# sringe/CatINT

Measured on AMD Instinct MI355X. Metric: batched 1D PNP Newton-timesteps/sec, higher is better.
Workload: dtype f64; 1 GPU; BASELINE configs[1]: batch=1024 operating points/GPU, 3 species, 512 grid points, fp64, Crank-Nicolson compat integrator, Dirichlet-Dirichlet Poisson; batch_per_gpu=1024, nspecies=3, nx=512, steps_per_launch=256, parallelism=batch-sharded x1

## Files before the change

### catint_amd/csrc/pnp_kernels.hip

```cpp
#include "pnp_internal.h"
#include "pnp_wave.h"

namespace pnp {

template <int P, bool WANT_V, int SHIFT, bool DD = false>
__device__ __forceinline__ double poisson_wave(const DevArgs& A, double* LV, double* GV, double* VV, double* X,
                                               double vw, double vb, double gw, double gb, int lane) {
  const int nx = A.nx, m = A.m;
  const int r0 = lane * P;
  const double dx = A.dx;
  double vown[P], gown[P];
  double v1;
  if constexpr (!WANT_V && P >= 2) {
    if (DD || A.pb_mode == PNP_PB_DD) {
      double Hi[P];
      const double dx2 = A.dx2;
      double s0 = 0.0, s1 = 0.0;
      double hm1, hm2, h0, h1, incT, incW;
      if constexpr (DD) {
        if (lane == 0) LV[pidx<P>(nx - 1)] = 0.0;
        lds_sync();
        {
#pragma clang fp contract(off)
#pragma unroll
          for (int j = 0; j < P; ++j) Hi[j] = LV[pidx<P>(r0 + j + 1)] * dx2;
          hm1 = LV[pidx<P>(m)] * dx2;
          hm2 = LV[pidx<P>(m - 1)] * dx2;
          h0 = LV[pidx<P>(1)] * dx2;
          h1 = LV[pidx<P>(2)] * dx2;
        }
#pragma unroll
        for (int j = 0; j < P; ++j) {
          s0 += Hi[j];
          s1 = __builtin_fma((double)j, Hi[j], s1);
        }
      } else {
#pragma unroll
        for (int j = 0; j < P; ++j) {
          double h = LV[pidx<P>(r0 + j + 1)] * dx2;
          h = (r0 + j == m) ? 0.0 : h;
          Hi[j] = h;
          s0 += h;
          s1 = __builtin_fma((double)j, h, s1);
        }
        hm1 = pick_blocked<P>(Hi, r0, m - 1);
        hm2 = pick_blocked<P>(Hi, r0, m - 2);
        h0 = read_lane(Hi[0], 0);
        h1 = read_lane(Hi[1], 0);
      }
      const double wsum = __builtin_fma((double)(m - r0), s0, -s1);
#pragma unroll
      for (int j = 1; j < P; ++j) Hi[j] += Hi[j - 1];
      if constexpr (DD) {
        incT = wave_scan_incl_bc(Hi[P - 1]);
        incW = wave_scan_incl_bc(wsum);
      } else {
        incT = wave_scan_incl(Hi[P - 1]);
        incW = wave_scan_incl(wsum);
      }
      const double base = from_prev_lane(0.0, incT);
      const double tot1 = read_lane(incT, 63), totG = read_lane(incW, 63);
#pragma unroll
      for (int j = 0; j < P; ++j) Hi[j] += base;
      const double w0 = (vb - vw - totG) / A.nxm1;
      const double inv2dx = A.inv2dx;
#pragma unroll
      for (int j = 0; j < P; ++j) {
        const double Hx = (j == 0) ? base : Hi[j > 0 ? j - 1 : 0];
        GV[pidx<P>(r0 + j + 1 + SHIFT)] = inv2dx * ((w0 + Hi[j]) + (w0 + Hx));
      }
      const double g1 = inv2dx * ((w0 + h0) + (w0 + 0.0));
      const double g2 = inv2dx * ((w0 + (h0 + h1)) + (w0 + h0));
      const double g_first = g1 + (g1 - g2);
      const double Hm1 = tot1 - hm1, Hm2 = Hm1 - hm2;
      const double gm1 = inv2dx * ((w0 + tot1) + (w0 + Hm1));
      const double gm2 = inv2dx * ((w0 + Hm1) + (w0 + Hm2));
      const double g_last = gm1 + (gm1 - gm2);
      lds_sync();
      if (lane == 0) {
        GV[pidx<P>(0 + SHIFT)] = g_first;
        GV[pidx<P>(nx - 1 + SHIFT)] = g_last;
        if constexpr (SHIFT == 1) {
          GV[pidx<P>(0)] = g_first;
          GV[pidx<P>(nx + 1)] = g_last;
          if constexpr (DD) GV[pidx<P>(nx - 2 + 1)] = g_last;
        }
      }
      lds_sync();
      return vw + w0;
    }
  }
  if (A.pb_mode == PNP_PB_DD) {
    double Hi[P];
    const double dx2 = dx * dx;
    if (lane == 0) LV[pidx<P>(nx - 1)] = 0.0;
    lds_sync();
#pragma unroll
    for (int j = 0; j < P; ++j) Hi[j] = LV[pidx<P>(r0 + j + 1)] * dx2;
    double tot1, baseH, totG;
    const double inv2dx = 1.0 / (2 * dx);
    if constexpr (!WANT_V) {
      double wsum = 0.0;
      const double wj0 = (double)(m - r0);
#pragma unroll
      for (int j = 0; j < P; ++j) wsum = __builtin_fma(wj0 - (double)j, Hi[j], wsum);
      blocked_scan_sum<P>(Hi, wsum, X, lane, tot1, baseH, totG);
    } else {
      double G[P];
      blocked_scan<P, false>(Hi, X, lane, tot1, baseH);
#pragma unroll
      for (int j = 0; j < P; ++j) G[j] = Hi[j];
      double totAll, baseG;
      blocked_scan<P, false>(G, X, lane, totAll, baseG);
      totG = totAll - (double)(64 * P - m) * tot1;
      const double w0v = (vb - vw - totG) / (double)(nx - 1);
#pragma unroll
      for (int j = 0; j < P; ++j) {
        const double Gex = (j == 0) ? baseG : G[j > 0 ? j - 1 : 0];
        vown[j] = vw + (double)(r0 + j + 1) * w0v + Gex;
      }
    }
    const double w0 = (vb - vw - totG) / (double)(nx - 1);
#pragma unroll
    for (int j = 0; j < P; ++j) {
      const double Hx = (j == 0) ? baseH : Hi[j > 0 ? j - 1 : 0];
      gown[j] = inv2dx * ((w0 + Hi[j]) + (w0 + Hx));
    }
    v1 = vw + 1.0 * w0 + 0.0;
  } else {
    const bool g_from_wall = (A.pb_mode == PNP_PB_GWALL_VBULK) || (A.pb_mode == PNP_PB_VWALL_GWALL);
    const bool v_from_wall = (A.pb_mode == PNP_PB_VWALL_GBULK) || (A.pb_mode == PNP_PB_VWALL_GWALL);
    double t[P];
#pragma unroll
    for (int j = 0; j < P; ++j) {
      const double lv = LV[pidx<P>(r0 + j + 1)];
      t[j] = (r0 + j < m) ? lv * dx : 0.0;
    }
    double tot, base;
    if (g_from_wall) {
      blocked_scan<P, false>(t, X, lane, tot, base);
#pragma unroll
      for (int j = 0; j < P; ++j) gown[j] = gw + t[j];
    } else {
      blocked_scan<P, true>(t, X, lane, tot, base);
#pragma unroll
      for (int j = 0; j < P; ++j) gown[j] = gb - t[j];
    }
#pragma unroll
    for (int j = 0; j < P; ++j) t[j] = (r0 + j < m) ? gown[j] * dx : 0.0;
    if (v_from_wall) {
      blocked_scan<P, false>(t, X, lane, tot, base);
#pragma unroll
      for (int j = 0; j < P; ++j) vown[j] = vw + t[j];
    } else {
      blocked_scan<P, true>(t, X, lane, tot, base);
#pragma unroll
      for (int j = 0; j < P; ++j) vown[j] = vb - t[j];
    }
    v1 = __shfl(vown[0], 0, 64);
  }
#pragma unroll
  for (int j = 0; j < P; ++j) {
    GV[pidx<P>(r0 + j + 1 + SHIFT)] = gown[j];
    if constexpr (WANT_V) VV[pidx<P>(r0 + j + 1)] = vown[j];
  }
  lds_sync();
  if (lane == 0) {
    const double g1 = GV[pidx<P>(1 + SHIFT)], g2 = GV[pidx<P>(2 + SHIFT)];
    const double gm1 = GV[pidx<P>(nx - 2 + SHIFT)], gm2 = GV[pidx<P>(nx - 3 + SHIFT)];
    double g0, gl;
    if (A.pb_mode == PNP_PB_DD) {
      g0 = g1 + (g1 - g2);
      gl = gm1 + (gm1 - gm2);
    } else if (A.pb_mode == PNP_PB_GWALL_VBULK || A.pb_mode == PNP_PB_VWALL_GWALL) {
      g0 = gw;
      gl = gm1 + (gm1 - gm2);
    } else {
      gl = gb;
      g0 = g1 + (g1 - g2);
    }
    GV[pidx<P>(0 + SHIFT)] = g0;
    GV[pidx<P>(nx - 1 + SHIFT)] = gl;
    if constexpr (SHIFT == 1) {
      GV[pidx<P>(0)] = g0;
      GV[pidx<P>(nx + 1)] = gl;
    }
    if constexpr (WANT_V) {
      const double v1 = VV[pidx<P>(1)], v2 = VV[pidx<P>(2)];
      const double vm1 = VV[pidx<P>(nx - 2)], vm2 = VV[pidx<P>(nx - 3)];
      double v0, vl;
      if (A.pb_mode == PNP_PB_DD) {
        v0 = vw;
        vl = vb;
      } else if (A.pb_mode == PNP_PB_VWALL_GBULK || A.pb_mode == PNP_PB_VWALL_GWALL) {
        v0 = vw;
        vl = vm1 + (vm1 - vm2);
      } else {
        vl = vb;
        v0 = v1 + (v1 - v2);
      }
      VV[pidx<P>(0)] = v0;
      VV[pidx<P>(nx - 1)] = vl;
    }
  }
  lds_sync();
  return v1;
}

template <int P, int G>
constexpr int step_min_waves() {
  return P <= 2 ? 4 : (P == 4 ? (G == 1 ? 4 : 2) : (P == 8 ? (G == 1 ? 3 : 1) : 1));
}

__device__ __forceinline__ double uniform_f64(double v) {
  const int lo = __builtin_amdgcn_readfirstlane(__double2loint(v));
  const int hi = __builtin_amdgcn_readfirstlane(__double2hiint(v));
  return __hiloint2double(hi, lo);
}

template <int P, int W, int G, bool FAST>
__device__ __forceinline__ void step_body(const DevArgs& A, double* lds) {
  constexpr int RB = rowbuf_doubles<P>();
  constexpr int NR = W * G;
  constexpr int V1SLOT = RB - 2;
  constexpr int IT2 = P / (2 * W) + 1;
  const int tid = threadIdx.x;
  const int lane = tid & 63;
  const int wave = __builtin_amdgcn_readfirstlane(tid >> 6);
  const int64_t b = blockIdx.x;
  const int nx = A.nx, m = A.m, ldx = A.ldx, N = A.N;
  double* LV = lds;
  double* GV = lds + RB;
  double* ROWS = lds + 2 * RB;
  double* ROW0 = ROWS + wave * (G * RB);
  const int r0 = lane * P;
  const double dx = A.dx, dt = A.dt;

  double* lin = A.lapl_a + b * (int64_t)ldx;
  double* lout = A.lapl_b + b * (int64_t)ldx;
  double* crow0 = A.c + b * (int64_t)N * ldx;
  const bool single_round = FAST || (N <= NR);
  const bool cn = FAST || (A.method == PNP_METHOD_CRANK_NICOLSON);
  const bool use_mig = FAST || A.use_mig;
  double chk = 0.0;
  double mn = 0.0;
  for (int i = tid; i < (2 + NR) * RB; i += 64 * W) lds[i] = 0.0;
  wg_sync<W>();
  const int ls2 = pidx<P>(2 * tid);
  const bool lead_all = W > 1 && wave == 0 && A.B <= 2048;
  if (lead_all) __builtin_amdgcn_s_setprio(3);

  auto stage_first_round = [&]() {
    RowRegs<P> rl, rr[G];
    if (wave == 0 && use_mig) load_row_issue<P>(row_rsrc(lin, ldx), rl, lane);
    if (wave * G < N) {
#pragma unroll
      for (int g = 0; g < G; ++g)
        load_row_issue<P>(row_rsrc(crow0 + (int64_t)min(wave * G + g, N - 1) * ldx, ldx), rr[g], lane);
    }
    if (wave == 0 && use_mig) load_row_commit<P>(rl, LV, lane);
    if (wave * G < N) {
#pragma unroll
      for (int g = 0; g < G; ++g) load_row_commit<P>(rr[g], ROW0 + g * RB, lane);
    }
    lds_sync();
  };

  double k_vw = 0.0, k_vb = 0.0, k_vz = 0.0;
  double k_f2dx[G], k_cL[G], k_mu[G], k_twoD[G], k_hsr[G], k_e4r[G], k_eer[G], k_omsr[G], k_qe[NR];
  if constexpr (FAST) {
    k_vw = uniform_f64(A.pb[b * 4 + 0]);
    k_vb = uniform_f64(A.pb[b * 4 + 1]);
    k_vz = uniform_f64(A.vzeta[b]);
#pragma unroll
    for (int g = 0; g < G; ++g) {
      const int k = min(wave * G + g, N - 1);
      const SpecConst& S = A.spec[k];
      k_f2dx[g] = uniform_f64(2 * A.flux[b * N + k] * dx);
      k_cL[g] = uniform_f64(A.cbulk[b * N + k]);
      k_mu[g] = uniform_f64(S.mu);
      k_twoD[g] = uniform_f64(S.twoD);
      k_hsr[g] = uniform_f64(S.hsr);
      k_e4r[g] = uniform_f64(S.e4r);
      k_eer[g] = uniform_f64(S.eer);
      k_omsr[g] = uniform_f64(S.omsr);
    }
#pragma unroll
    for (int w2 = 0; w2 < NR; ++w2) k_qe[w2] = uniform_f64(A.spec[min(w2, N - 1)].qe);
    stage_first_round();
  }

  for (int step = 0; step < A.nsteps; ++step) {
    const bool resident = single_round && step > 0;
    const bool last_step = step + 1 == A.nsteps;
    if constexpr (!FAST) {
      if (!resident) stage_first_round();
    }
    __builtin_amdgcn_sched_barrier(0);
    if (use_mig) {
      if (wave == 0) {
        const double vw = FAST ? k_vw : A.pb[b * 4 + 0], vb = FAST ? k_vb : A.pb[b * 4 + 1];
        const double gw = FAST ? 0.0 : A.pb[b * 4 + 2], gb = FAST ? 0.0 : A.pb[b * 4 + 3];
        int lane_o = lane;
        asm volatile("" : "+v"(lane_o));
        if (W > 1 && !lead_all) __builtin_amdgcn_s_setprio(3);
        const double v1w = poisson_wave<P, false, 1, FAST>(A, LV, GV, nullptr, GV, vw, vb, gw, gb, lane_o);
        if (W > 1 && !lead_all) __builtin_amdgcn_s_setprio(0);
        if (lane == 0) {
          GV[V1SLOT] = v1w;
          if (!FAST && cn) GV[pidx<P>(nx - 2 + 1)] = GV[pidx<P>(nx - 1 + 1)];
        }
      }
    }
    wg_sync<W>();
    const double v1 = use_mig ? GV[V1SLOT] : 0.0;
    const double vz = FAST ? k_vz : A.vzeta[b];

    d2 accp[IT2];
#pragma unroll
    for (int it = 0; it < IT2; ++it) accp[it] = (d2)(0.0);

    for (int k0 = 0; k0 < N; k0 = FAST ? N : k0 + NR) {
      const int kw = k0 + wave * G;
      if (kw < N) {
        int kg[G];
#pragma unroll
        for (int g = 0; g < G; ++g) kg[g] = min(kw + g, N - 1);
        if (!FAST && k0 > 0) {
          RowRegs<P> rr[G];
#pragma unroll
          for (int g = 0; g < G; ++g) load_row_issue<P>(row_rsrc(crow0 + (int64_t)kg[g] * ldx, ldx), rr[g], lane);
#pragma unroll
          for (int g = 0; g < G; ++g) load_row_commit<P>(rr[g], ROW0 + g * RB, lane);
          lds_sync();
        }
        double c0new[G], cLv[G], pat0[G], patL[G];
#pragma unroll
        for (int g = 0; g < G; ++g) {
          const double* ROW = ROW0 + g * RB;
          const SpecConst& S = A.spec[kg[g]];
          const double flux = FAST ? 0.0 : A.flux[b * N + kg[g]];
          const double cL = FAST ? k_cL[g] : A.cbulk[b * N + kg[g]];
          const double c1 = ROW[pidx<P>(1)];
          const double c0old = ROW[pidx<P>(0)];
          const double cLold = ROW[pidx<P>(nx - 1)];
          double aa;
          if constexpr (FAST) {
#pragma clang fp contract(off)
            aa = k_mu[g] * (v1 - vz);
          } else {
            aa = S.mu * (v1 - vz);
          }
          if (cn) {
            const double twoD = FAST ? k_twoD[g] : S.twoD;
            const double rden = fast_rcp2(-twoD + aa);
            c0new[g] = (-twoD - aa) * rden * c1 - (FAST ? k_f2dx[g] : 2 * flux * dx) * rden;
          } else {
            c0new[g] = ((S.twoD + aa) * c1 + flux * 2. * dx) * fast_rcp2(S.twoD - aa);
          }
          cLv[g] = cL;
          pat0[g] = cn ? (c0new[g] + c0old) : c0new[g];
          patL[g] = cn ? (cL + cLold) : cL;
        }
        lds_sync();
        if (lane == 0) {
#pragma unroll
          for (int g = 0; g < G; ++g) {
            ROW0[g * RB + pidx<P>(0)] = pat0[g];
            ROW0[g * RB + pidx<P>(nx - 1)] = patL[g];
          }
        }
        lds_sync();
        double x[G][P];
        if (cn) {
          double ta[G][P], tc[G][P];
          {
            const int jmu = (m - 1) % P;
            const bool in_lm = lane == (m - 1) / P;
#pragma unroll
            for (int g = 0; g < G; ++g) {
              const double* ROW = ROW0 + g * RB;
              const SpecConst& S = A.spec[kg[g]];
              const double hsr = FAST ? k_hsr[g] : S.hsr, e4r = FAST ? k_e4r[g] : S.e4r;
              const double eer = FAST ? k_eer[g] : S.eer, omsr = FAST ? k_omsr[g] : S.omsr;
              double cc[P + 2], g4[P + 2];
#pragma unroll
              for (int t = 0; t < P + 2; ++t) cc[t] = ROW[pidx<P>(r0 + t)];
#pragma unroll
              for (int t = 0; t < P + 2; ++t) g4[t] = e4r * GV[pidx<P>(r0 + t)];
#pragma unroll
              for (int j = 0; j < P; ++j) {
                const double lq = LV[pidx<P>(r0 + j)];
                const double left = cc[j] * (hsr + g4[j]);
                const double right = cc[j + 2] * (hsr - g4[j + 2]);
                x[g][j] = left + cc[j + 1] * (omsr + eer * lq) + right;
                ta[g][j] = -hsr + g4[j + 1];
                tc[g][j] = -hsr - g4[j + 1];
                if (j == jmu) tc[g][j] = in_lm ? 0.0 : tc[g][j];
              }
              if (lane == 0) ta[g][0] = 0.0;
            }
          }
          __builtin_amdgcn_sched_barrier(0);
          lds_sync();
          tridiag_wave<P, G, FAST>(ta, tc, x, ROW0, RB, lane);
        } else {
          double gq[P + 2];
#pragma unroll
          for (int t = 0; t < P + 2; ++t) gq[t] = A.use_mig ? GV[pidx<P>(r0 + t + 1)] : 0.0;
#pragma unroll
          for (int g = 0; g < G; ++g) {
            const double* ROW = ROW0 + g * RB;
            const SpecConst& S = A.spec[kg[g]];
            const double sf = S.sf, dm = S.dm, Mf = S.Mf;
            double cc[P + 2];
#pragma unroll
            for (int t = 0; t < P + 2; ++t) cc[t] = ROW[pidx<P>(r0 + t)];
#pragma unroll
            for (int j = 0; j < P; ++j) {
              double Wt = sf - dm * gq[j + 2] + 0.5;
              double Et = sf + dm * gq[j] + 0.5;
              if (!A.lf) {
                Wt -= 0.5;
                Et -= 0.5;
              }
              double val = __builtin_fma(Wt, cc[j + 2], __builtin_fma(Mf, cc[j + 1], Et * cc[j]));
              if (A.has_rates) val += A.rates[(b * N + kg[g]) * (int64_t)ldx + min(r0 + j + 1, nx - 1)] * dt;
              x[g][j] = val;
            }
          }
          lds_sync();
        }
#pragma unroll
        for (int g = 0; g < G; ++g) {
          double* ROW = ROW0 + g * RB;
#pragma unroll
          for (int j = 0; j < P; ++j) ROW[pidx<P>(r0 + j + 1)] = x[g][j];
        }
        lds_sync();
#pragma unroll
        for (int g = 0; g < G; ++g) {
          double* ROW = ROW0 + g * RB;
          if (lane == 0) {
            ROW[pidx<P>(0)] = c0new[g];
            ROW[pidx<P>(nx - 1)] = cLv[g];
          }
          if (lane < ldx - nx) ROW[pidx<P>(nx + lane)] = 0.0;
        }
      }
      wg_sync<W>();
      const int nk = min(NR, N - k0);
      auto store_and_fold = [&](int w2, double qe) {
        const double* R2 = ROWS + w2 * RB;
        double* grow = crow0 + (int64_t)(k0 + w2) * ldx;
        const __amdgpu_buffer_rsrc_t rs = row_rsrc(grow, ldx);
#pragma unroll
        for (int it = 0; it < IT2; ++it) {
          if (FAST && W > 1 && it > 0 && 128 * (W * it + wave) >= ldx) continue;
          const int sl = min(pair_slot<P>(ls2, W * it), RB - 4);
          d2 t;
          t.x = R2[sl];
          t.y = R2[sl + PAIR_STEP<P>];
          __builtin_amdgcn_raw_buffer_store_b128(__builtin_bit_cast(u4, t), rs, tid * 16 + it * (1024 * W), 0, 0);
          accp[it].x = __builtin_fma(-t.x, qe, accp[it].x);
          accp[it].y = __builtin_fma(-t.y, qe, accp[it].y);
          if (last_step) {
            const bool inrow = 2 * tid + 128 * W * it < ldx;
            const double sx = inrow ? t.x : 0.0, sy = inrow ? t.y : 0.0;
            chk += (sx - sx) + (sy - sy);
            mn = fmin(mn, fmin(sx, sy));
          }
        }
      };
      if constexpr (FAST) {
#pragma unroll
        for (int w2 = 0; w2 < NR; ++w2)
          if (w2 < nk) store_and_fold(w2, k_qe[w2]);
      } else {
        for (int w2 = 0; w2 < nk; ++w2) store_and_fold(w2, A.spec[k0 + w2].qe);
        wg_sync<W>();
      }
    }
    const bool keep = single_round && (step + 1 < A.nsteps);
    {
      const __amdgpu_buffer_rsrc_t rs = row_rsrc(lout, ldx);
#pragma unroll
      for (int it = 0; it < IT2; ++it) {
        if (FAST && W > 1 && it > 0 && 128 * (W * it + wave) >= ldx) continue;
        __builtin_amdgcn_raw_buffer_store_b128(__builtin_bit_cast(u4, accp[it]), rs, tid * 16 + it * (1024 * W), 0, 0);
        if (keep && 2 * tid + 128 * W * it < ldx) {
          LV[pair_slot<P>(ls2, W * it)] = accp[it].x;
          LV[pair_slot<P>(ls2, W * it) + PAIR_STEP<P>] = accp[it].y;
        }
      }
    }
    double* tmp = lin;
    lin = lout;
    lout = tmp;
    if (step + 1 < A.nsteps) {
      if (single_round) {
        wg_sync<W>();
      } else {
        __builtin_amdgcn_fence(__ATOMIC_RELEASE, "workgroup");
        if constexpr (W > 1) __builtin_amdgcn_s_barrier();
        __builtin_amdgcn_fence(__ATOMIC_ACQUIRE, "workgroup");
      }
    }
  }
  const unsigned long long nan_mask = __ballot(chk != chk);
  const unsigned long long neg_mask = __ballot(mn < 0.0);
  if (lane == 0) {
    int st = PNP_STATUS_OK;
    if (neg_mask) st = PNP_STATUS_NEGATIVE;
    if (nan_mask) st = PNP_STATUS_NAN;
    if (st) atomicMax(&A.status[b], st);
#ifdef PNP_HWID_PROBE
    const unsigned simd = __builtin_amdgcn_s_getreg((1 << 11) | (4 << 6) | 4);
    unsigned v = 1u << (8 + 4 * wave + simd);
    if (wave == 0) v |= (__builtin_amdgcn_s_getreg((3 << 11) | (8 << 6) | 4) << 20) | (__builtin_amdgcn_s_getreg((2 << 11) | (13 << 6) | 4) << 24);
    atomicOr((unsigned*)&A.status[b], v);
#endif
  }
}

template <int P, int W, int G>
constexpr bool step_has_fast_body() {
  return P >= 2 && !(W == 1 && G == 3 && (P == 2 || P == 16));
}

template <int P, int W, int G>
__global__ __launch_bounds__(64 * W, (step_min_waves<P, G>())) void step_kernel(const DevArgs A) {
  extern __shared__ __attribute__((aligned(16))) double lds[];
  if constexpr (step_has_fast_body<P, W, G>()) {
    const bool fast = A.method == PNP_METHOD_CRANK_NICOLSON && A.use_mig && A.pb_mode == PNP_PB_DD && !A.has_rates &&
                      A.N <= W * G && !A.step_generic;
    if (fast) {
      step_body<P, W, G, true>(A, lds);
      return;
    }
  }
  step_body<P, W, G, false>(A, lds);
}

template <int P, int W>
constexpr int step_rr_min_waves() {
  return P <= 4 ? 4 : (P == 8 ? 3 : 1);
}

template <int P, int W, bool CN>
__global__ __launch_bounds__(64 * W, (step_rr_min_waves<P, W>())) void step_kernel_rr(const DevArgs A) {
  static_assert(P >= 2 && P % 2 == 0, "window loads need an even P");
  extern __shared__ __attribute__((aligned(16))) double lds[];
  constexpr int XS = 384;
  constexpr int PS = 64 * P + 2;
  const int tid = threadIdx.x;
  const int lane = tid & 63;
  const int wave = __builtin_amdgcn_readfirstlane(tid >> 6);
  const int64_t b = blockIdx.x;
  const int nx = A.nx, m = A.m, ldx = A.ldx, N = A.N;
  const int r0 = lane * P;
  const double dx = A.dx;
  constexpr bool cn = CN;
  double* strip = lds + wave * XS;
  double* part = lds + W * XS;
  double* lin = A.lapl_a + b * (int64_t)ldx;
  double* lout = A.lapl_b + b * (int64_t)ldx;
  double* crow0 = A.c + b * (int64_t)N * ldx;
  const double vw = A.pb[b * 4 + 0], vb = A.pb[b * 4 + 1];
  const double vz = A.vzeta[b];
  const bool single_round = (N <= W);
  double chk = 0.0, mn = 0.0;

  double lw[P + 2];
  double cc[P + 2];
  for (int step = 0; step < A.nsteps; ++step) {
    const bool last_step = step + 1 == A.nsteps;
    const bool resident = single_round && step > 0;
    if (!resident) {
      if (A.use_mig) load_window<P>(row_rsrc(lin, ldx), lw, lane);
      load_window<P>(row_rsrc(crow0 + (int64_t)min(wave, N - 1) * ldx, ldx), cc, lane);
    }
    double gx[P + 3];
    double v1 = 0.0;
    if (A.use_mig) {
      double Hi[P];
      const double dx2 = dx * dx;
      double s0 = 0.0, s1 = 0.0;
#pragma unroll
      for (int j = 0; j < P; ++j) {
        double h = lw[j + 1] * dx2;
        h = (r0 + j == m) ? 0.0 : h;
        Hi[j] = h;
        s0 += h;
        s1 = __builtin_fma((double)j, h, s1);
      }
      const double wsum = __builtin_fma((double)(m - r0), s0, -s1);
      const double hm1 = pick_blocked<P>(Hi, r0, m - 1), hm2 = pick_blocked<P>(Hi, r0, m - 2);
      const double h0 = read_lane(Hi[0], 0), h1 = read_lane(Hi[1], 0);
#pragma unroll
      for (int j = 1; j < P; ++j) Hi[j] += Hi[j - 1];
      const double incT = wave_scan_incl(Hi[P - 1]);
      const double incW = wave_scan_incl(wsum);
      const double base = from_prev_lane(0.0, incT);
      const double tot1 = read_lane(incT, 63), totG = read_lane(incW, 63);
#pragma unroll
      for (int j = 0; j < P; ++j) Hi[j] += base;
      const double w0 = (vb - vw - totG) / (double)(nx - 1);
      v1 = vw + w0;
      const double inv2dx = 1.0 / (2 * dx);
      double gown[P];
#pragma unroll
      for (int j = 0; j < P; ++j) {
        const double Hx = (j == 0) ? base : Hi[j > 0 ? j - 1 : 0];
        gown[j] = inv2dx * ((w0 + Hi[j]) + (w0 + Hx));
      }
      const double g1 = inv2dx * ((w0 + h0) + (w0 + 0.0));
      const double g2 = inv2dx * ((w0 + (h0 + h1)) + (w0 + h0));
      const double g_first = g1 + (g1 - g2);
      const double Hm1 = tot1 - hm1, Hm2 = Hm1 - hm2;
      const double gm1 = inv2dx * ((w0 + tot1) + (w0 + Hm1));
      const double gm2 = inv2dx * ((w0 + Hm1) + (w0 + Hm2));
      const double g_last = gm1 + (gm1 - gm2);
#pragma unroll
      for (int t = 2; t < P + 2; ++t) gx[t] = gown[t - 2];
      gx[1] = from_prev_lane(g_first, gown[P - 1]);
      gx[0] = from_prev_lane(g_first, gown[P - 2]);
      gx[P + 2] = from_next_lane(0.0, gown[0]);
#pragma unroll
      for (int t = 2; t < P + 3; ++t) {
        const int idx = r0 - 1 + t;
        gx[t] = ((cn && idx == nx - 2) || idx == nx - 1) ? g_last : gx[t];
      }
    } else {
#pragma unroll
      for (int t = 0; t < P + 3; ++t) gx[t] = 0.0;
    }

    double acc[P];
#pragma unroll
    for (int j = 0; j < P; ++j) acc[j] = 0.0;
    double acc0 = 0.0, accL = 0.0;

    for (int k = wave; k < N; k += W) {
      if (k != wave) load_window<P>(row_rsrc(crow0 + (int64_t)k * ldx, ldx), cc, lane);
      const SpecConst& S = A.spec[k];
      const double flux = A.flux[b * N + k];
      const double cL = A.cbulk[b * N + k];
      const double c0old = read_lane(cc[0], 0);
      const double c1 = read_lane(cc[1], 0);
      const double aa = S.mu * (v1 - vz);
      double c0new;
      if (cn) {
        const double rden = fast_rcp2(-S.twoD + aa);
        c0new = (-S.twoD - aa) * rden * c1 - 2 * flux * dx * rden;
      } else {
        c0new = ((S.twoD + aa) * c1 + flux * 2. * dx) * fast_rcp2(S.twoD - aa);
      }
      const double qe = S.qe;
      const double pat0 = cn ? (c0new + c0old) : c0new;
      const double patL = cn ? (cL + cL) : cL;
      cc[0] = (lane == 0) ? pat0 : cc[0];
#pragma unroll
      for (int t = 2; t < P + 2; ++t) cc[t] = (r0 + t == nx - 1) ? patL : cc[t];
      double x[1][P];
      if (cn) {
        double ta[1][P], tc[1][P];
        const double hsr = S.hsr, e4r = S.e4r, eer = S.eer, omsr = S.omsr;
#pragma unroll
        for (int j = 0; j < P; ++j) {
          const double gm = e4r * gx[j], g0 = e4r * gx[j + 1], gp = e4r * gx[j + 2];
          const double left = cc[j] * (hsr + gm);
          const double right = cc[j + 2] * (hsr - gp);
          x[0][j] = left + cc[j + 1] * (omsr + eer * lw[j]) + right;
          ta[0][j] = -hsr + g0;
          tc[0][j] = (r0 + j == m - 1) ? 0.0 : (-hsr - g0);
        }
        ta[0][0] = (lane == 0) ? 0.0 : ta[0][0];
        tridiag_wave<P, 1>(ta, tc, x, strip, XS, lane);
      } else {
        const double sf = S.sf, dm = S.dm, Mf = S.Mf;
#pragma unroll
        for (int j = 0; j < P; ++j) {
          double Wt = sf - dm * gx[j + 3] + 0.5;
          double Et = sf + dm * gx[j + 1] + 0.5;
          if (!A.lf) {
            Wt -= 0.5;
            Et -= 0.5;
          }
          x[0][j] = Et * cc[j] + Mf * cc[j + 1] + Wt * cc[j + 2];
        }
      }
      double* grow = crow0 + (int64_t)k * ldx;
      store_rows<P>(__builtin_amdgcn_make_buffer_rsrc(grow, 0, (nx - 1) * 8, 0x00020000), x[0], lane);
      if (lane == 0) grow[0] = c0new;
#pragma unroll
      for (int j = 0; j < P; ++j) {
        const double xv = (r0 + j < m) ? x[0][j] : 0.0;
        acc[j] = __builtin_fma(-xv, qe, acc[j]);
        if (last_step) {
          chk += xv - xv;
          mn = fmin(mn, xv);
        }
      }
      if (last_step) {
        chk += c0new - c0new;
        mn = fmin(mn, c0new);
      }
      acc0 = __builtin_fma(-c0new, qe, acc0);
      accL = __builtin_fma(-cL, qe, accL);
      if (single_round) {
#pragma unroll
        for (int j = 0; j < P; ++j) cc[j + 1] = x[0][j];
        cc[0] = from_prev_lane(c0new, x[0][P - 1]);
        cc[P + 1] = from_next_lane(0.0, x[0][0]);
      }
    }
    if constexpr (W > 1) {
      double* mine = part + ((step & 1) * W + wave) * PS;
#pragma unroll
      for (int j = 0; j < P; ++j) mine[r0 + j] = acc[j];
      if (lane == 0) {
        mine[64 * P] = acc0;
        mine[64 * P + 1] = accL;
      }
      wg_sync<W>();
      const double* all = part + (step & 1) * W * PS;
#pragma unroll
      for (int j = 0; j < P; ++j) {
        double t = all[r0 + j];
#pragma unroll
        for (int w2 = 1; w2 < W; ++w2) t += all[w2 * PS + r0 + j];
        acc[j] = t;
      }
      double t0 = all[64 * P], tL = all[64 * P + 1];
#pragma unroll
      for (int w2 = 1; w2 < W; ++w2) {
        t0 += all[w2 * PS + 64 * P];
        tL += all[w2 * PS + 64 * P + 1];
      }
      acc0 = t0;
      accL = tL;
    }
    if (wave == 0) {
      const __amdgpu_buffer_rsrc_t rs = __builtin_amdgcn_make_buffer_rsrc(lout, 0, (nx - 1) * 8, 0x00020000);
      store_rows<P>(rs, acc, lane);
      if (lane == 0) {
        lout[0] = acc0;
        lout[nx - 1] = accL;
      }
    }
    if (single_round) {
#pragma unroll
      for (int j = 0; j < P; ++j) lw[j + 1] = acc[j];
      lw[0] = from_prev_lane(acc0, acc[P - 1]);
      lw[P + 1] = 0.0;
    }
    double* tmp = lin;
    lin = lout;
    lout = tmp;
    if (!single_round && step + 1 < A.nsteps) {
      __builtin_amdgcn_fence(__ATOMIC_RELEASE, "workgroup");
      if constexpr (W > 1) __builtin_amdgcn_s_barrier();
      __builtin_amdgcn_fence(__ATOMIC_ACQUIRE, "workgroup");
    }
  }
  const unsigned long long nan_mask = __ballot(chk != chk);
  const unsigned long long neg_mask = __ballot(mn < 0.0);
  if (lane == 0) {
    int st = PNP_STATUS_OK;
    if (neg_mask) st = PNP_STATUS_NEGATIVE;
    if (nan_mask) st = PNP_STATUS_NAN;
    if (st) atomicMax(&A.status[b], st);
  }
}

template <int P, int WY>
__host__ __device__ constexpr int rowbuf_mw_doubles() {
  constexpr int CAP = 128 * WY * (P / 2 + 1);
  return (CAP + CAP / P + 4 + 1) & ~1;
}
template <int WY>
__host__ __device__ constexpr int xch_doubles() {
  return 2 * 3 * (2 * 64 * WY);
}

template <int P, int WY, bool REV>
__device__ __forceinline__ void blocked_scan_wg(double (&x)[P], double* strip_w, double* tots, int lane, int wave,
                                                double& total, double& base) {
  double wt, wb;
  blocked_scan<P, REV>(x, strip_w, lane, wt, wb);
  if (lane == 0) tots[wave] = wt;
  wg_sync<2>();
  double off = 0.0, all = 0.0;
#pragma unroll
  for (int w2 = 0; w2 < WY; ++w2) {
    const double t = tots[w2];
    all += t;
    off += (REV ? (w2 > wave) : (w2 < wave)) ? t : 0.0;
  }
#pragma unroll
  for (int j = 0; j < P; ++j) x[j] += off;
  total = all;
  base = wb + off;
  wg_sync<2>();
}

template <int P, int WY, bool WANT_V, int SHIFT>
__device__ __forceinline__ double poisson_wg(const DevArgs& A, double* LV, double* GV, double* VV, double* strip_w,
// ... 856 lines not shown
```

Baseline: 261.5 million timesteps/s.

## Precompute CN stencil coefficients and restructure fast-path row store/fold loop

```diff
diff --git a/catint_amd/csrc/pnp_kernels.hip b/catint_amd/csrc/pnp_kernels.hip
--- a/catint_amd/csrc/pnp_kernels.hip
+++ b/catint_amd/csrc/pnp_kernels.hip
@@ -218,12 +218,18 @@
   return __hiloint2double(hi, lo);
 }
 
+template <int P, int W, int G>
+constexpr bool step_two_coefficients() {
+  return !(P == 4 && W >= 3) && !(P == 16 && W == 1 && G == 3);
+}
+
 template <int P, int W, int G, bool FAST>
 __device__ __forceinline__ void step_body(const DevArgs& A, double* lds) {
   constexpr int RB = rowbuf_doubles<P>();
   constexpr int NR = W * G;
   constexpr int V1SLOT = RB - 2;
   constexpr int IT2 = P / (2 * W) + 1;
+  constexpr bool TWO_COEF = step_two_coefficients<P, W, G>();
   const int tid = threadIdx.x;
   const int lane = tid & 63;
   const int wave = __builtin_amdgcn_readfirstlane(tid >> 6);
@@ -383,20 +389,40 @@
               const SpecConst& S = A.spec[kg[g]];
               const double hsr = FAST ? k_hsr[g] : S.hsr, e4r = FAST ? k_e4r[g] : S.e4r;
               const double eer = FAST ? k_eer[g] : S.eer, omsr = FAST ? k_omsr[g] : S.omsr;
-              double cc[P + 2], g4[P + 2];
+              double cc[P + 2];
 #pragma unroll
               for (int t = 0; t < P + 2; ++t) cc[t] = ROW[pidx<P>(r0 + t)];
-#pragma unroll
-              for (int t = 0; t < P + 2; ++t) g4[t] = e4r * GV[pidx<P>(r0 + t)];
-#pragma unroll
-              for (int j = 0; j < P; ++j) {
-                const double lq = LV[pidx<P>(r0 + j)];
-                const double left = cc[j] * (hsr + g4[j]);
-                const double right = cc[j + 2] * (hsr - g4[j + 2]);
-                x[g][j] = left + cc[j + 1] * (omsr + eer * lq) + right;
-                ta[g][j] = -hsr + g4[j + 1];
-                tc[g][j] = -hsr - g4[j + 1];
-                if (j == jmu) tc[g][j] = in_lm ? 0.0 : tc[g][j];
+              if constexpr (TWO_COEF) {
+                double sp[P + 1], sm[P + 2];
+#pragma unroll
+                for (int t = 0; t < P + 2; ++t) {
+                  const double gv = GV[pidx<P>(r0 + t)];
+                  if (t <= P) sp[t] = __builtin_fma(e4r, gv, hsr);
+                  sm[t] = __builtin_fma(-e4r, gv, hsr);
+                }
+#pragma unroll
+                for (int j = 0; j < P; ++j) {
+                  const double lq = LV[pidx<P>(r0 + j)];
+                  const double mid = cc[j + 1] * __builtin_fma(eer, lq, omsr);
+                  x[g][j] = __builtin_fma(cc[j + 2], sm[j + 2], __builtin_fma(cc[j], sp[j], mid));
+                  ta[g][j] = -sm[j + 1];
+                  tc[g][j] = -sp[j + 1];
+                  if (j == jmu) tc[g][j] = in_lm ? 0.0 : tc[g][j];
+                }
+              } else {
+                double g4[P + 2];
+#pragma unroll
+                for (int t = 0; t < P + 2; ++t) g4[t] = e4r * GV[pidx<P>(r0 + t)];
+#pragma unroll
+                for (int j = 0; j < P; ++j) {
+                  const double lq = LV[pidx<P>(r0 + j)];
+                  const double left = cc[j] * (hsr + g4[j]);
+                  const double right = cc[j + 2] * (hsr - g4[j + 2]);
+                  x[g][j] = left + cc[j + 1] * (omsr + eer * lq) + right;
+                  ta[g][j] = -hsr + g4[j + 1];
+                  tc[g][j] = -hsr - g4[j + 1];
+                  if (j == jmu) tc[g][j] = in_lm ? 0.0 : tc[g][j];
+                }
               }
               if (lane == 0) ta[g][0] = 0.0;
             }
@@ -456,7 +482,6 @@
         const __amdgpu_buffer_rsrc_t rs = row_rsrc(grow, ldx);
 #pragma unroll
         for (int it = 0; it < IT2; ++it) {
-          if (FAST && W > 1 && it > 0 && 128 * (W * it + wave) >= ldx) continue;
           const int sl = min(pair_slot<P>(ls2, W * it), RB - 4);
           d2 t;
           t.x = R2[sl];
@@ -474,8 +499,25 @@
       };
       if constexpr (FAST) {
 #pragma unroll
-        for (int w2 = 0; w2 < NR; ++w2)
-          if (w2 < nk) store_and_fold(w2, k_qe[w2]);
+        for (int it = 0; it < IT2; ++it) {
+          if (W > 1 && it > 0 && 128 * (W * it + wave) >= ldx) continue;
+          const int sl = min(pair_slot<P>(ls2, W * it), RB - 4);
+          d2 t[NR];
+#pragma unroll
+          for (int w2 = 0; w2 < NR; ++w2) {
+            t[w2].x = ROWS[w2 * RB + sl];
+            t[w2].y = ROWS[w2 * RB + sl + PAIR_STEP<P>];
+          }
+#pragma unroll
+          for (int w2 = 0; w2 < NR; ++w2) {
+            if (w2 < nk) {
+              const __amdgpu_buffer_rsrc_t rs = row_rsrc(crow0 + (int64_t)w2 * ldx, ldx);
+              __builtin_amdgcn_raw_buffer_store_b128(__builtin_bit_cast(u4, t[w2]), rs, tid * 16 + it * (1024 * W), 0, 0);
+              accp[it].x = __builtin_fma(-t[w2].x, k_qe[w2], accp[it].x);
+              accp[it].y = __builtin_fma(-t[w2].y, k_qe[w2], accp[it].y);
+            }
+          }
+        }
       } else {
         for (int w2 = 0; w2 < nk; ++w2) store_and_fold(w2, A.spec[k0 + w2].qe);
         wg_sync<W>();
@@ -504,6 +546,21 @@
         __builtin_amdgcn_fence(__ATOMIC_RELEASE, "workgroup");
         if constexpr (W > 1) __builtin_amdgcn_s_barrier();
         __builtin_amdgcn_fence(__ATOMIC_ACQUIRE, "workgroup");
+      }
+    }
+  }
+  if constexpr (FAST) {
+    if (A.nsteps > 0) {
+      const int nk = min(NR, N);
+      for (int w2 = 0; w2 < nk; ++w2) {
+#pragma unroll
+        for (int it = 0; it < IT2; ++it) {
+          const int sl = min(pair_slot<P>(ls2, W * it), RB - 4);
+          const bool inrow = 2 * tid + 128 * W * it < ldx;
+          const double sx = inrow ? ROWS[w2 * RB + sl] : 0.0, sy = inrow ? ROWS[w2 * RB + sl + PAIR_STEP<P>] : 0.0;
+          chk += (sx - sx) + (sy - sy);
+          mn = fmin(mn, fmin(sx, sy));
+        }
       }
     }
   }
```

New measurement: 268.0 million timesteps/s (median of 6 runs). +2.5%, better.
